# UnaryPlus/raytrace

Measured on AMD Instinct MI355X. Metric: Msamples/s (pixels×spp/s) + achieved HBM GB/s, Cornell-box 600×600, higher is better.
Workload: dtype f64; 1 GPU; cornell 600x600 200spp depth 50; width=600, height=600, spp=200, max_depth=50, parallelism=rows interleaved over 1 GPU(s), row_block 1

## Files before the change

### raytrace_amd/csrc/rt_trace.h

```cpp
#ifndef RT_TRACE_COMMON_H
#define RT_TRACE_COMMON_H
#include <stdint.h>

#include "../../include/rt.h"
#include "rt_internal.h"
#include "rt_sincos_table.h"

#ifdef RT_HOST_EMU
#include <cmath>
#include <cstring>
#define RT_FN static inline
#define RT_FN_SPEC inline
namespace rt_emu {
inline int f2i(float f) {
  int i;
  std::memcpy(&i, &f, 4);
  return i;
}
extern thread_local long long counters[4];
}
#define RT_F2I(f) rt_emu::f2i(f)
#define RT_COUNT(i) (++rt_emu::counters[i])
#define RT_ANY(x) (x)
#define RT_BALLOT_COUNT(x) ((x) ? 1 : 0)
#define RT_CAS
#else
#define RT_FN __device__ __forceinline__
#define RT_FN_SPEC __device__ __forceinline__
#define RT_F2I(f) __float_as_int(f)
#define RT_COUNT(i) ((void)0)
#define RT_ANY(x) __any(x)
#define RT_BALLOT_COUNT(x) ((int)__popcll(__ballot(x)))
#define RT_CAS __attribute__((address_space(4)))
#endif

#ifndef RT_HOOK_SEGMENT
#define RT_HOOK_SEGMENT(pix, sample, seg, R, tbest, best, hit_medium, L, T)
#endif
#ifndef RT_HOOK_SAMPLE
#define RT_HOOK_SAMPLE(pix, sample, L)
#endif
#endif

#ifndef RT_F64
#define RT_F64 0
#endif
#undef RT_NS
#undef RL
#undef RMIN
#undef RMAX
#undef RABS
#undef RFLOOR
#undef RCOPYSIGN
#undef RATAN2
#undef RACOS
#undef RSIN
#undef RFMA
#undef RT_NAN
#undef RT_HUGE
#undef RT_R2I
#undef RT_SINCOS_TURNS
#undef RT_SINCOS_TURNS_S
#undef RT_LOG
#undef RT_RSQRT
#undef RT_RCP
#undef RT_RCP_NZ
#undef RT_SQRT
#undef RT_NODE_F32
#if RT_F64
#define RT_NS rtk64
#define RL(x) x
#define RMIN fmin
#define RMAX fmax
#define RABS fabs
#define RFLOOR floor
#define RCOPYSIGN copysign
#define RATAN2 atan2
#define RACOS acos
#define RSIN sin
#define RFMA fma
#define RT_NAN __builtin_nan("")
#define RT_HUGE __builtin_huge_val()
#define RT_R2I(x) ((int)(uint32_t)__builtin_bit_cast(unsigned long long, (double)(x)))
#define RT_LOG(x) log(x)
#if defined(RT_HOST_EMU) || defined(RT_MATH64_IEEE)
#define RT_SINCOS_TURNS(x, s, c) (*(s) = sin(6.283185307179586 * (x)), *(c) = cos(6.283185307179586 * (x)))
#define RT_RSQRT(x) (1.0 / sqrt(x))
#define RT_RCP(x) (1.0 / (x))
#define RT_RCP_NZ(x) (1.0 / (x))
#define RT_SQRT(x) sqrt(x)
#else
#define RT_SINCOS_TURNS(x, s, c) rt_math64::sincos_turns(x, s, c)
#define RT_SINCOS_TURNS_S(x, s, c) rt_math64::sincos_turns<true>(x, s, c)
#define RT_RSQRT(x) rt_math64::rsqrt(x)
#define RT_RCP(x) rt_math64::rcp(x)
#define RT_RCP_NZ(x) rt_math64::rcp_nz(x)
#define RT_SQRT(x) rt_math64::sqrt_nonneg(x)
#ifndef RT_MATH64_DEFINED
#define RT_MATH64_DEFINED
namespace rt_math64 {
__device__ __forceinline__ double rcp(double x) {
  const double r0 = __builtin_amdgcn_rcp(x);
  const double e = __builtin_fma(-x, r0, 1.0);
  const double r = __builtin_fma(r0, __builtin_fma(e, e, e), r0);
  return r == r ? r : r0;
}
__device__ __forceinline__ double rcp_nz(double x) {
  const double r0 = __builtin_amdgcn_rcp(x);
  const double e = __builtin_fma(-x, r0, 1.0);
  return __builtin_fma(r0, __builtin_fma(e, e, e), r0);
}
__device__ __forceinline__ double rsqrt(double x) {
  const double y = __builtin_amdgcn_rsq(x);
  const double e = __builtin_fma(-x * y, y, 1.0);
  return __builtin_fma(y, __builtin_fma(e, 0.375, 0.5) * e, y);
}
__device__ __forceinline__ double sqrt_nonneg(double x) {
  const double y = __builtin_amdgcn_rsq(x);
  double s = x * y, h = 0.5 * y;
  const double r = __builtin_fma(-s, h, 0.5);
  s = __builtin_fma(s, r, s);
  h = __builtin_fma(h, r, h);
  const double d = __builtin_fma(-s, s, x);
  s = __builtin_fma(d, h, s);
  return x == 0.0 || x == __builtin_huge_val() ? x : s;
}
}
#endif
#endif
#ifndef RT_MATH64_SINCOS_DEFINED
#define RT_MATH64_SINCOS_DEFINED
#ifdef RT_HOST_EMU
#define RT_MATH64_FN static inline
#define RT_MATH64_TAB static
#else
#define RT_MATH64_FN __device__ __forceinline__
#define RT_MATH64_TAB __device__
#endif
namespace rt_math64 {
RT_MATH64_TAB const double rt_sincos_tab[2 * RT_SINCOS_TABLE_N] = RT_SINCOS_TABLE_INIT;
template <bool kCoefScalar = false>
RT_MATH64_FN void sincos_turns(double u, double* sn, double* cs) {
  const double kq = __builtin_rint(u * (double)RT_SINCOS_TABLE_N);
  const double b = __builtin_fma(kq, -1.0 / RT_SINCOS_TABLE_N, u);
  const int k = (int)kq & (RT_SINCOS_TABLE_N - 1);
  const double sa = rt_sincos_tab[2 * k], ca = rt_sincos_tab[2 * k + 1];
  const double x = b * 6.283185307179586, x2 = x * x;
  double c120 = 1.0 / 120.0;
#ifndef RT_HOST_EMU
  if constexpr (kCoefScalar) asm volatile("" : "+s"(c120));
#endif
  double ps = __builtin_fma(x2, -1.0 / 5040.0, c120);
  ps = __builtin_fma(x2, ps, -1.0 / 6.0);
  const double sb = __builtin_fma(x2 * x, ps, x);
  double pc = __builtin_fma(x2, -1.0 / 720.0, 1.0 / 24.0);
  pc = __builtin_fma(x2, pc, -0.5);
  const double cb = __builtin_fma(x2, pc, 1.0);
  *sn = __builtin_fma(sa, cb, ca * sb);
  *cs = __builtin_fma(ca, cb, -(sa * sb));
}
}
#endif
#else
#define RT_NS rtk
#define RL(x) x##f
#define RMIN fminf
#define RMAX fmaxf
#define RABS fabsf
#define RFLOOR floorf
#define RCOPYSIGN copysignf
#define RATAN2 atan2f
#define RACOS acosf
#define RSIN sinf
#define RFMA fmaf
#define RT_NAN __builtin_nanf("")
#define RT_HUGE __builtin_huge_valf()
#define RT_R2I(x) RT_F2I(x)
#ifdef RT_HOST_EMU
#define RT_SINCOS_TURNS(x, s, c) (*(s) = sinf(6.283185307179586f * (x)), *(c) = cosf(6.283185307179586f * (x)))
#define RT_LOG(x) logf(x)
#define RT_RSQRT(x) (1.0f / sqrtf(x))
#define RT_RCP(x) (1.0f / (x))
#define RT_RCP_NZ(x) (1.0f / (x))
#define RT_SQRT(x) sqrtf(x)
#else
#define RT_SINCOS_TURNS(x, s, c) (*(s) = __builtin_amdgcn_sinf(x), *(c) = __builtin_amdgcn_cosf(x))
#define RT_LOG(x) __logf(x)
#define RT_RSQRT(x) __frsqrt_rn(x)
#define RT_RCP(x) __builtin_amdgcn_rcpf(x)
#define RT_RCP_NZ(x) __builtin_amdgcn_rcpf(x)
#define RT_SQRT(x) __builtin_amdgcn_sqrtf(x)
#endif
#endif

namespace RT_NS {

#if RT_F64
using real = double;
using ureal = unsigned long long;
#else
using real = float;
using ureal = uint32_t;
#endif
using KernelParams = ::KernelParamsT<real>;
using DevMaterial = ::DevMaterialT<real>;
using DevTexture = ::DevTextureT<real>;
using DevMedium = ::DevMediumT<real>;
using DevBox = ::DevBoxT<real>;
using DevTarget = ::DevTargetT<real>;
using DevCamera = ::DevCameraT<real>;
using DevInstance = ::DevInstanceT<real>;



constexpr real kPi = RL(3.14159265358979323846);
constexpr real kTmin = RL(0.0001);
constexpr real kInf = RT_HUGE;

#ifdef RT_HOST_EMU
struct alignas(16) v4 {
#else
struct alignas(4 * sizeof(real)) v4 {
#endif
  real x, y, z, w;
};
struct alignas(16) v4f {
  float x, y, z, w;
};
struct alignas(16) i4 {
  int x, y, z, w;
};
struct f3 {
  real x, y, z;
};
RT_FN f3 mk3(real x, real y, real z) { return f3{x, y, z}; }
RT_FN f3 ld3(const real* p) { return f3{p[0], p[1], p[2]}; }
RT_FN f3 operator+(f3 a, f3 b) { return f3{a.x + b.x, a.y + b.y, a.z + b.z}; }
RT_FN f3 operator-(f3 a, f3 b) { return f3{a.x - b.x, a.y - b.y, a.z - b.z}; }
RT_FN f3 operator-(f3 a) { return f3{-a.x, -a.y, -a.z}; }
RT_FN f3 operator*(real s, f3 a) { return f3{s * a.x, s * a.y, s * a.z}; }
RT_FN f3 operator*(f3 a, f3 b) { return f3{a.x * b.x, a.y * b.y, a.z * b.z}; }
RT_FN real dot(f3 a, f3 b) { return a.x * b.x + a.y * b.y + a.z * b.z; }
RT_FN f3 normalize(f3 v) {
  real l = dot(v, v);
#if RT_F64
  if (RABS(l) <= RL(1e-12) || RABS(RL(1.0) - l) <= RL(1e-12)) return v;
#else
  if (l <= RL(1e-12)) return v;
#endif
  return RT_RSQRT(l) * v;
}
RT_FN f3 unit(f3 v) { return RT_RSQRT(dot(v, v)) * v; }
RT_FN f3 reflect(f3 n, f3 v) { return v - (RL(2.0) * dot(n, v)) * n; }
RT_FN f3 xyz(v4 v) { return f3{v.x, v.y, v.z}; }
RT_FN v4 ld4(const real* p) { return *reinterpret_cast<const v4*>(p); }
typedef const RT_CAS real* cfp;
RT_FN cfp cf(const real* p) { return (cfp)p; }
RT_FN f3 ldc3(cfp p) { return f3{p[0], p[1], p[2]}; }
RT_FN v4 ldc4(cfp p) {
  const RT_CAS v4* q = (const RT_CAS v4*)p;
  return v4{q->x, q->y, q->z, q->w};
}
RT_FN int ldci(const int* p, int i) { return ((const RT_CAS int*)p)[i]; }
typedef const RT_CAS float* cfpf;
RT_FN v4f ldc4f(cfpf p) {
  const RT_CAS v4f* q = (const RT_CAS v4f*)p;
  return v4f{q->x, q->y, q->z, q->w};
}

struct u4 {
  uint32_t x, y, z, w;
};
#ifdef RT_HOST_EMU
#define RT_XOR3(a, b, c) ((a) ^ (b) ^ (c))
#else
#define RT_XOR3(a, b, c) __builtin_amdgcn_bitop3_b32((a), (b), (c), 0x96)
#endif
RT_FN u4 philox(uint32_t c0, uint32_t c1, uint32_t c2, uint32_t c3, uint32_t k0, uint32_t k1) {
#ifndef RT_PHILOX_ROUNDS
#define RT_PHILOX_ROUNDS 10
#endif
#ifndef RT_HOST_EMU
  asm volatile("" : "+s"(k0), "+s"(k1));
#endif
#pragma unroll
  for (int r = 0; r < RT_PHILOX_ROUNDS; ++r) {
    if (r) {
      k0 += 0x9E3779B9u;
      k1 += 0xBB67AE85u;
    }
    const uint64_t p0 = (uint64_t)0xD2511F53u * c0, p1 = (uint64_t)0xCD9E8D57u * c2;
    const uint32_t hi0 = (uint32_t)(p0 >> 32), lo0 = (uint32_t)p0;
    const uint32_t hi1 = (uint32_t)(p1 >> 32), lo1 = (uint32_t)p1;
    uint32_t n0 = RT_XOR3(hi1, c1, k0), n2 = RT_XOR3(hi0, c3, k1);
    c0 = n0;
    c1 = lo1;
    c2 = n2;
    c3 = lo0;
  }
  return u4{c0, c1, c2, c3};
}
RT_FN real u01(uint32_t w) { return (real)(w >> 8) * (RL(1.0) / RL(16777216.0)); }

#ifndef RT_SINCOS_TURNS_S
#define RT_SINCOS_TURNS_S RT_SINCOS_TURNS
#endif
template <bool kFlatLoop = false>
RT_FN f3 unit_vector(uint32_t a, uint32_t b) {
  real z = RL(1.0) - RL(2.0) * u01(a);
  real r = RT_SQRT(RMAX(RL(0.0), RL(1.0) - z * z));
  real s, c;
  if constexpr (kFlatLoop)
    RT_SINCOS_TURNS_S(u01(b), &s, &c);
  else
    RT_SINCOS_TURNS(u01(b), &s, &c);
  return mk3(r * c, r * s, z);
}

#if RT_F64 && !defined(RT_NODE_F64)
#define RT_NODE_F32 1
struct f3n {
  float x, y, z;
};
#else
#define RT_NODE_F32 0
#endif
struct RayCtx {
  f3 o, d;
#if RT_NODE_F32
  f3n idir, off0, off1;
#else
  f3 idir, oidir;
#endif
  uint32_t time_w;
  int self_gid;
  int self_inst;
};
template <bool kInst>
RT_FN bool is_self(const RayCtx& R, int gid, int cur_inst) {
  if constexpr (kInst) return gid == R.self_gid && cur_inst == R.self_inst;
  return gid == R.self_gid;
}

RT_FN real u01(uint32_t w);
RT_FN f3 motion_shift(const KernelParams& P, int m, uint32_t time_w) {
  const real time = u01(time_w);
  f3 v0 = ldc3(cf(P.motions) + 8 * m), v1 = ldc3(cf(P.motions) + 8 * m + 4);
  return (RL(1.0) - time) * v0 + time * v1;
}

RT_FN real safe_rcp(real d) { return RT_RCP(RABS(d) > RL(1e-20) ? d : RCOPYSIGN(RL(1e-20), d)); }

#if RT_NODE_F32
#ifndef RT_RCPF
#ifdef RT_HOST_EMU
#define RT_RCPF(x) (1.0f / (x))
#else
#define RT_RCPF(x) __builtin_amdgcn_rcpf(x)
#endif
#endif
RT_FN void prep_axis(real o, real d, float& fi, float& f0, float& f1) {
#ifndef RT_NODE_RCP64
  const float i = RT_RCPF((float)(RABS(d) > RL(1e-20) ? d : RCOPYSIGN(RL(1e-20), d)));
  const float oi = (float)(o * (real)i);
#else
  const real i = safe_rcp(d);
  const float oi = (float)(o * i);
#endif
  const float pad = 3.0e-7f * fabsf(oi);
  const float sp = i >= 0 ? pad : -pad;
  fi = (float)i;
  f0 = oi + sp;
  f1 = oi - sp;
}
RT_FN void prep_ray(RayCtx& R) {
  prep_axis(R.o.x, R.d.x, R.idir.x, R.off0.x, R.off1.x);
  prep_axis(R.o.y, R.d.y, R.idir.y, R.off0.y, R.off1.y);
  prep_axis(R.o.z, R.d.z, R.idir.z, R.off0.z, R.off1.z);
}
RT_FN void node_slabs_f32(const RayCtx& R, const v4f& n0, const v4f& n1, const v4f& n2, float tminf, float ctf,
                          float& lnear, float& lfar, float& rnear, float& rfar) {
  const float lx0 = fmaf(n0.x, R.idir.x, -R.off0.x), lx1 = fmaf(n0.y, R.idir.x, -R.off1.x);
  const float ly0 = fmaf(n0.z, R.idir.y, -R.off0.y), ly1 = fmaf(n0.w, R.idir.y, -R.off1.y);
  const float lz0 = fmaf(n2.x, R.idir.z, -R.off0.z), lz1 = fmaf(n2.y, R.idir.z, -R.off1.z);
  const float rx0 = fmaf(n1.x, R.idir.x, -R.off0.x), rx1 = fmaf(n1.y, R.idir.x, -R.off1.x);
  const float ry0 = fmaf(n1.z, R.idir.y, -R.off0.y), ry1 = fmaf(n1.w, R.idir.y, -R.off1.y);
  const float rz0 = fmaf(n2.z, R.idir.z, -R.off0.z), rz1 = fmaf(n2.w, R.idir.z, -R.off1.z);
  lnear = fmaxf(fmaxf(fminf(lx0, lx1), fminf(ly0, ly1)), fmaxf(fminf(lz0, lz1), tminf));
  lfar = fminf(fminf(fmaxf(lx0, lx1), fmaxf(ly0, ly1)), fminf(fmaxf(lz0, lz1), ctf)) * 1.00000095f;
  rnear = fmaxf(fmaxf(fminf(rx0, rx1), fminf(ry0, ry1)), fmaxf(fminf(rz0, rz1), tminf));
  rfar = fminf(fminf(fmaxf(rx0, rx1), fmaxf(ry0, ry1)), fminf(fmaxf(rz0, rz1), ctf)) * 1.00000095f;
}
#else
RT_FN void prep_ray(RayCtx& R) {
  R.idir = mk3(safe_rcp(R.d.x), safe_rcp(R.d.y), safe_rcp(R.d.z));
  R.oidir = R.o * R.idir;
}
#endif

RT_FN const RT_CAS DevInstance* inst_rec(const KernelParams& P, int k) { return (const RT_CAS DevInstance*)P.instances + k; }
RT_FN f3 inst_to_object(const RT_CAS DevInstance* I, f3 v, bool point) {
  if (point) v = v - mk3(I->m[3], I->m[7], I->m[11]);
  return mk3(I->m[0] * v.x + I->m[4] * v.y + I->m[8] * v.z, I->m[1] * v.x + I->m[5] * v.y + I->m[9] * v.z,
             I->m[2] * v.x + I->m[6] * v.y + I->m[10] * v.z);
}
RT_FN f3 inst_rotate(const RT_CAS DevInstance* I, f3 v) {
  return mk3(I->m[0] * v.x + I->m[1] * v.y + I->m[2] * v.z, I->m[4] * v.x + I->m[5] * v.y + I->m[6] * v.z,
             I->m[8] * v.x + I->m[9] * v.y + I->m[10] * v.z);
}

#if RT_F64
struct Closest {
  real t;
  int ord;
  int prim;
  int inst;
};
#else
struct Closest {
  real t;
  unsigned long long key;
  int prim;
  int inst;
};
#endif
struct Trav {
  int* stack;
  int stride;
  const v4f* lds_nodes;
};
#if RT_F64
RT_FN Closest no_hit() { return Closest{kInf, 0, -1, -1}; }
#else
RT_FN Closest no_hit() { return Closest{kInf, 0x7f80000000000000ull, -1, -1}; }
RT_FN unsigned long long hit_key(real t, int ord) {
  return ((unsigned long long)(unsigned)RT_F2I(t) << 32) | (unsigned)ord;
}
#endif

struct PrimRec {
  v4 a, b, c, e;
};
RT_FN PrimRec ld_rec(cfp pr) { return PrimRec{ldc4(pr), ldc4(pr + 4), ldc4(pr + 8), ldc4(pr + 12)}; }
#ifdef RT_HOST_EMU
#define RT_REC_ALIGN 16
#else
#define RT_REC_ALIGN (16 * sizeof(real))
#endif
struct alignas(RT_REC_ALIGN) PrimRec64 {
  real f[16];
};
RT_FN PrimRec ld_rec64(const RT_CAS PrimRec64* p) {
  const RT_CAS real* r = p->f;
  return PrimRec{v4{r[0], r[1], r[2], r[3]}, v4{r[4], r[5], r[6], r[7]}, v4{r[8], r[9], r[10], r[11]},
                 v4{r[12], r[13], r[14], r[15]}};
}

#if RT_F64
RT_FN real float_up(real x) { return __builtin_bit_cast(real, __builtin_bit_cast(long long, x) + 1); }
#else
RT_FN real float_up(real x) { return __builtin_bit_cast(real, RT_F2I(x) + 1); }
#endif
RT_FN void isect_sphere(const PrimRec& r, f3 o, const RayCtx& R, real tmin, real tmin_up, bool self, real& t,
                        real& q) {
  f3 oc = xyz(r.a) - o;
// ... 609 lines not shown
template <bool kInst, class RC>
RT_FN void test_leaf_generic(const KernelParams& P, RC& R, TravState& S) {
  while (S.leaf < 0) {
    const int enc = ~S.leaf;
    const int first = enc >> RT_LEAF_SHIFT, count = (enc & ((1 << RT_LEAF_SHIFT) - 1)) + 1;
    for (int k = 0; k < count; ++k)
      test_rec<false, kInst>(P, ld_rec(cf(P.prims) + 16 * (size_t)(first + k)), first + k, R, S.tmin, S.tmin_up, S.C,
                             S.inst, S.ord_base);
    S.leaf = 0;
  }
}

template <bool kDefer>
RT_FN void closest_flat(const KernelParams& P, int set, const RayCtx& R, real tmin, Closest& C, real* apdf = nullptr) {
  {
    const DevFlatSet& S = P.flat_sets[set];
    const real tmin_up = float_up(tmin);
    for (int b = S.box_first; b < S.box_end; ++b) test_box<true>((const RT_CAS DevBox*)P.boxes + b, R, tmin_up, C);
    int k = S.first;
    const RT_CAS PrimRec64* rp = (const RT_CAS PrimRec64*)P.flat_recs + k;
    for (; k < S.end_quad; ++k, ++rp) {
      if constexpr (kDefer) {
        if (k == P.target_rec) {
          real term;
          test_static<RT_PRIM_CLASS_QUAD>(ld_rec64(rp), R, tmin, tmin_up, C, 0, &term);
          *apdf = RFMA(P.targets[0].prob_icr, term, *apdf);
          continue;
        }
      }
      test_static<RT_PRIM_CLASS_QUAD>(ld_rec64(rp), R, tmin, tmin_up, C);
    }
    for (; k < S.end_tri; ++k, ++rp) test_static<RT_PRIM_CLASS_TRI>(ld_rec64(rp), R, tmin, tmin_up, C);
    for (; k < S.end_sphere; ++k, ++rp) test_static<RT_PRIM_CLASS_SPHERE>(ld_rec64(rp), R, tmin, tmin_up, C);
    for (; k < S.end; ++k, ++rp) test_rec<true>(P, ld_rec64(rp), k, R, tmin, tmin_up, C);
#if RT_F64
    if (C.t < kInf) C.prim = C.ord;
#else
    const uint32_t hi = (uint32_t)(C.key >> 32);
    if (hi < 0x7f800000u) {
      C.t = __builtin_bit_cast(real, hi);
      C.prim = (int)(uint32_t)C.key;
    }
#endif
  }
}
template <>
RT_FN_SPEC void closest<true>(const KernelParams& P, cfp prims, int root, int set, const RayCtx& R, real tmin, Closest& C,
                         const Trav& W, int* overflow) {
  (void)prims;
  (void)root;
  (void)W;
  (void)overflow;
  closest_flat<false>(P, set, R, tmin, C);
}

template <>
RT_FN_SPEC void closest<false>(const KernelParams& P, cfp prims, int root, int set, const RayCtx& R, real tmin,
                          Closest& C, const Trav& W, int* overflow) {
  TravState S;
  trav_begin(S, root, tmin);
  if (set == 0) prefix_hits(P, prims, R, tmin, S.C);
  while (!trav_done(S)) trav_round(P, R, S, W, *overflow RT_PROF_NULLARG);
  C = S.C;
}

#ifndef RT_KARGS_OPAQUE
#define RT_KARGS_OPAQUE 1
#endif
#if defined(RT_HOST_EMU) || !RT_KARGS_OPAQUE
#define RT_KARGS(P0) (P0)
#else
RT_FN const KernelParams& rt_kargs() {
  const RT_CAS KernelParams* pp = (const RT_CAS KernelParams*)__builtin_amdgcn_kernarg_segment_ptr();
  asm volatile("" : "+s"(pp));
  return *(const KernelParams*)pp;
}
#define RT_KARGS(P0) rt_kargs()
#endif
#ifndef RT_KARGS_TRAV
#define RT_KARGS_TRAV RT_F64
#endif
#define RT_KARGS_IF(on, P0) ((on) ? RT_KARGS(P0) : (P0))

RT_FN uint32_t fast_div(uint32_t n, const FastDiv& f) {
  if (f.d == 1u) return n;
  const uint32_t t = (uint32_t)(((uint64_t)n * f.m) >> 32);
  return (t + ((n - t) >> 1)) >> f.s;
}
RT_FN void camera_ray(const KernelParams& P, uint32_t pix, int sample, uint32_t pxgy, RayCtx& R) {
  int gy, px;
  if (pxgy == ~0u) {
    gy = (int)fast_div(pix, P.div_width);
    px = (int)pix - gy * P.cam.width;
  } else {
    gy = (int)(pxgy >> 16);
    px = (int)(pxgy & 0xffffu);
  }
  u4 w0 = philox(pix, (uint32_t)sample, 0u, RT_EV_CAMERA0, P.key0, P.key1);
  R.time_w = w0.z;
  f3 origin = ld3(P.cam.center);
  if (P.cam.disk_u[0] != RL(0.0) || P.cam.disk_u[1] != RL(0.0) || P.cam.disk_u[2] != RL(0.0) || P.cam.disk_v[0] != RL(0.0) ||
      P.cam.disk_v[1] != RL(0.0) || P.cam.disk_v[2] != RL(0.0)) {
    u4 w1 = philox(pix, (uint32_t)sample, 0u, RT_EV_CAMERA1, P.key0, P.key1);
    real rad = RT_SQRT(u01(w0.w)), s, c;
    RT_SINCOS_TURNS(u01(w1.x), &s, &c);
    origin = origin + (rad * c) * ld3(P.cam.disk_u) + (rad * s) * ld3(P.cam.disk_v);
  }
  f3 target = ld3(P.cam.top_left) + ((real)px + u01(w0.x)) * ld3(P.cam.pixel_u) +
              ((real)gy + u01(w0.y)) * ld3(P.cam.pixel_v);
  R.o = origin;
  R.d = normalize(target - origin);
  R.self_gid = -1;
  R.self_inst = -1;
}

RT_FN void medium_draw(const KernelParams& P, int m, u4 wm, real lo, real hi, real& tbest, int& hit_medium) {
#ifndef RT_HOST_EMU
#pragma clang fp contract(off)
#endif
  uint32_t wsel = (m & 3) == 0 ? wm.x : (m & 3) == 1 ? wm.y : (m & 3) == 2 ? wm.z : wm.w;
  real rnd = RL(1.0) - u01(wsel);
  real hit_dist = P.media[m].neg_inv_density * RT_LOG(rnd);
  if (hit_dist < hi - lo) {
    real t = lo + hit_dist;
    if (t < tbest) {
      tbest = t;
      hit_medium = m;
    }
  }
}
RT_FN u4 medium_block(const KernelParams& P, int m, uint32_t pix, int sample, int seg) {
  return philox(pix, (uint32_t)sample, (uint32_t)seg, RT_EV_MEDIA + (uint32_t)(m >> 2), P.key0, P.key1);
}
RT_FN void medium_event(const KernelParams& P, int m, uint32_t pix, int sample, int seg, real lo, real hi,
                        real& tbest, int& hit_medium) {
  medium_draw(P, m, medium_block(P, m, pix, sample, seg), lo, hi, tbest, hit_medium);
}

template <bool kMats, bool kEarly, class... Defer>
RT_FN bool mixture_scatter(const KernelParams& P, const HitInfo& h, const RayCtx& R, const u4& w, const DevMaterial& Mt,
                           bool hemi, f3 tex, f3& newdir, f3& Tf, Defer... apdf) {
  constexpr bool kDefer = sizeof...(Defer) == 1;
  real cr = u01(w.x);
  int choice = -1;
  for (int k = 0; k < P.n_targets; ++k) {
    if (cr < P.targets[k].thresh) {
      choice = k;
      break;
    }
  }
  f3 dir;
  if constexpr (kDefer) {
    if (choice < 0) {
      dir = h.n + unit_vector<true>(w.y, w.z);
    } else {
      const DevTarget& Tg = P.targets[choice];
      f3 lp = ld3(Tg.q) + u01(w.y) * ld3(Tg.u) + u01(w.z) * ld3(Tg.v);
      dir = lp - h.p;
    }
    dir = normalize(dir);
  } else if (choice < 0) {
    f3 uu = unit_vector(w.y, w.z);
    dir = hemi ? normalize(h.n + uu) : uu;
  } else {
    const DevTarget& Tg = P.targets[choice];
    f3 lp = ld3(Tg.q) + u01(w.y) * ld3(Tg.u) + u01(w.z) * ld3(Tg.v);
    dir = normalize(lp - h.p);
  }
  real pdf1 = hemi ? dot(dir, h.n) * (RL(1.0) / kPi) : RL(0.25) / kPi;
  if constexpr (kEarly)
    if (hemi && pdf1 <= RL(0.0)) return false;
  if constexpr (kDefer && !kMats && !kEarly) {
    if (P.target_defer) {
      *(apdf, ...) = P.rem_prob * pdf1;
      Tf = pdf1 * tex;
      newdir = dir;
      return !(hemi && pdf1 <= RL(0.0));
    }
  }
  real mix = RL(0.0);
  for (int k = 0; k < P.n_targets; ++k) {
    real tt, rinv;
    if (target_hit(P.targets[k], h.p, dir, tt, rinv)) mix += P.targets[k].prob_icr * (tt * tt * RABS(rinv));
  }
  real pdf = P.rem_prob * pdf1 + mix;
  f3 f = tex;
  if constexpr (kMats) {
    if (Mt.kind == 3) {
      real mu0 = -dot(R.d, h.n), mu1 = dot(dir, h.n);
      f = (RL(0.25) * RT_RCP(mu0 + mu1)) * f;
    } else if (Mt.kind == 9) {
      real g = Mt.param, mu = dot(R.d, dir);
      real base = RL(1.0) + g * g - RL(2.0) * g * mu;
      f = ((RL(1.0) - g * g) * RT_RCP(base * RT_SQRT(base))) * f;
    }
  }
  Tf = (pdf1 * RT_RCP(pdf)) * f;
  newdir = dir;
  return !(hemi && pdf1 <= RL(0.0));
}

template <int kTex, bool kMats, bool kInst, class... Defer>
RT_FN bool shade_event(const KernelParams& P, cfp prims, uint32_t pix, int sample, int seg, real tbest, int best,
                       int hit_medium, const RayCtx& R, f3& L, const f3& T, int best_inst, f3& np, f3& nd, f3& Tf,
                       int& ngid, Defer... apdf) {
  RT_HOOK_SEGMENT(pix, sample, seg, R, tbest, best, hit_medium, L, T);
  if (hit_medium < 0 && best < 0) {
    f3 bg = ld3(P.cam.bg0);
    if (P.cam.bg_kind == 1) {
      real a = RL(0.5) * (R.d.y + RL(1.0));
      bg = (RL(1.0) - a) * bg + a * ld3(P.cam.bg1);
    }
    L = L + T * bg;
#ifndef RT_HOST_EMU
    Tf = bg;
#endif
    return true;
  }
  bool terminate = false;
  const RT_CAS DevMaterial* Mp = hit_medium >= 0
                                     ? (const RT_CAS DevMaterial*)P.mats + P.media[hit_medium].material
                                     : (const RT_CAS DevMaterial*)P.prim_shade + best;
  if constexpr (kInst) {
    if (hit_medium < 0 && best_inst >= 0) {
      const int im = inst_rec(P, best_inst)->material;
      if (im >= 0) Mp = (const RT_CAS DevMaterial*)P.mats + im;
    }
  }
  const DevMaterial Mt = DevMaterial{Mp->kind, Mp->tex, Mp->param, Mp->tex_const, {RL(0.), RL(0.), RL(0.)}, RL(0.)};
  const bool need_tex = kTex > 0 && !Mt.tex_const && Mt.kind != RT_MAT_PITCH_BLACK && Mt.kind != RT_MAT_DIELECTRIC;
  HitInfo h;
  if (hit_medium >= 0) {
    h.p = R.o + tbest * R.d;
    h.n = -R.d;
    h.front = true;
    h.u = RL(0.);
    h.v = RL(0.);
    h.gid = -1;
  } else {
    if constexpr (kInst) {
      if (best_inst >= 0) {
        const RT_CAS DevInstance* I = inst_rec(P, best_inst);
        RayCtx Ro = R;
        Ro.o = inst_to_object(I, R.o, true);
        Ro.d = inst_to_object(I, R.d, false);
        h = surface_info(P, prims, best, Ro, tbest, need_tex);
        h.p = R.o + tbest * R.d;
        h.n = inst_rotate(I, h.n);
      } else {
        h = surface_info(P, prims, best, R, tbest, need_tex);
      }
    } else {
      h = surface_info(P, prims, best, R, tbest, need_tex);
    }
  }
  f3 tex = f3{Mp->c0[0], Mp->c0[1], Mp->c0[2]};
  if (need_tex) tex = eval_texture<kTex == 2>(P, Mt.tex, h.u, h.v, h.p);
  u4 w = philox(pix, (uint32_t)sample, (uint32_t)seg, RT_EV_SCATTER, P.key0, P.key1);
#ifdef RT_HOST_EMU
  f3 newdir = mk3(RT_NAN, RT_NAN, RT_NAN);
#elif defined(RT_SHADE_UNDEF)
  f3 newdir;
#else
  f3 newdir = R.d;
  Tf = tex;
#endif
  if constexpr (!kMats) {
    if (Mt.kind == 0) L = L + T * tex;
    terminate = !mixture_scatter<false, false>(P, h, R, w, Mt, true, tex, newdir, Tf, apdf...) || Mt.kind < 2;
  } else {
    switch (Mt.kind) {
      case 0:
        L = L + T * tex;
        terminate = true;
        break;
      case 1:
        terminate = true;
        break;
      case 4:
        Tf = tex;
        newdir = unit(reflect(h.n, R.d));
        break;
      case 5: {
        f3 d2 = reflect(h.n, R.d) + Mt.param * unit_vector(w.y, w.z);
        if (dot(d2, h.n) > RL(0.0)) {
          Tf = tex;
          newdir = normalize(d2);
        } else {
          terminate = true;
        }
        break;
      }
      case 6: {
        Tf = mk3(RL(1.), RL(1.), RL(1.));
        real ior = Mt.param;
        real ratio = h.front ? RT_RCP(ior) : ior;
        real cos_t = RMIN(RL(1.0), -dot(h.n, R.d));
        real sin_t = RT_SQRT(RMAX(RL(0.0), RL(1.0) - cos_t * cos_t));
        real r0 = (RL(1.0) - ratio) * RT_RCP(RL(1.0) + ratio);
        r0 = r0 * r0;
        real x1 = RL(1.0) - cos_t, x2 = x1 * x1;
        real reflectance = r0 + (RL(1.0) - r0) * (x2 * x2 * x1);
        if (ratio * sin_t > RL(1.0) || u01(w.x) < reflectance) {
          newdir = unit(reflect(h.n, R.d));
        } else {
          f3 perp = ratio * (R.d + cos_t * h.n);
          newdir = unit(perp - RT_SQRT(RABS(RL(1.0) - dot(perp, perp))) * h.n);
        }
        break;
      }
      case 7:
        Tf = tex;
        newdir = R.d;
        break;
      default:
        terminate = !mixture_scatter<true, true>(P, h, R, w, Mt, Mt.kind == 2 || Mt.kind == 3, tex, newdir, Tf);
        break;
    }
  }
  np = h.p;
  nd = newdir;
  ngid = h.gid;
  return terminate;
}
template <int kTex, bool kMats, bool kInst = false, class... Defer>
RT_FN bool shade(const KernelParams& P, cfp prims, uint32_t pix, int sample, int& seg, real tbest, int best,
                 int hit_medium, RayCtx& R, f3& L, f3& T, int best_inst = -1, Defer... apdf) {
#ifdef RT_HOST_EMU
  const real nan = RT_NAN;
  f3 np = mk3(nan, nan, nan), nd = np, Tf = np;
  int ngid = RT_EMPTY_ROOT;
#elif defined(RT_SHADE_UNDEF)
  f3 np, nd, Tf;
  int ngid;
#else
  f3 np = R.o, nd = R.d, Tf = mk3(RL(1.), RL(1.), RL(1.));
  int ngid = R.self_gid;
#endif
  const bool term =
      shade_event<kTex, kMats, kInst>(P, prims, pix, sample, seg, tbest, best, hit_medium, R, L, T, best_inst, np, nd, Tf,
                                      ngid, apdf...);
  R.o = np;
  R.d = nd;
  T = T * Tf;
  R.self_gid = ngid;
  if constexpr (kInst) R.self_inst = hit_medium >= 0 ? -1 : best_inst;
  const bool cont = !term && seg + 1 < P.cam.max_depth;
  ++seg;
  return !cont;
}

struct ItemCtx {
  int tp;
  int sample, s_end;
  uint32_t pix;
  uint32_t pxgy;
};
template <bool kTwoSizes>
RT_FN bool open_item(const KernelParams& P, int item, ItemCtx& I) {
  const int W = P.cam.width;
  const bool big = kTwoSizes && item < P.big_items;
  const int id = kTwoSizes && !big ? item - P.big_items : item;
  const int n = big ? P.n_big_chunks : P.n_chunks;
  I.tp = (int)fast_div((uint32_t)id, big ? P.div_big : P.div_small);
  const int k = id - I.tp * n;
  const int tr = (int)fast_div((uint32_t)I.tp, P.div_width);
  const int px = I.tp - tr * W;
  const int tb = (int)fast_div((uint32_t)tr, P.div_block);
  const int gy = (tb * P.n_shards + P.shard) * P.row_block + (tr - tb * P.row_block);
  I.pix = (uint32_t)(gy * W + px);
  I.pxgy = (uint32_t)gy << 16 | (uint32_t)px;
  const int chunk = big ? P.big_chunk : P.chunk;
  I.sample = P.sample0 + (big || !kTwoSizes ? 0 : P.small_start) + k * chunk;
  const int last = P.sample0 + P.cam.spp;
  I.s_end = I.sample + chunk < last ? I.sample + chunk : last;
  if (gy >= P.cam.height || P.cam.max_depth <= 0) I.s_end = I.sample;
  return I.sample < I.s_end;
}

#ifndef RT_TAIL_STEAL
#define RT_TAIL_STEAL 1
#endif
#ifndef RT_TAIL_STEAL_BVH
#define RT_TAIL_STEAL_BVH 1
#endif
#if (RT_TAIL_STEAL || RT_TAIL_STEAL_BVH) && !defined(RT_HOST_EMU)
RT_FN bool steal_sample(bool thief, ItemCtx& I, int tp_plain) {
  unsigned long long tm = __ballot(thief);
  unsigned long long vm = __ballot(!thief && I.tp != -1 && I.s_end - I.sample >= 2);
  const int lane = (int)__lane_id();
  bool got = false;
  while (tm != 0ull && vm != 0ull) {
    const int t = __ffsll(tm) - 1, v = __ffsll(vm) - 1;
    tm &= tm - 1ull;
    vm &= vm - 1ull;
    const int s_end = __builtin_amdgcn_readlane(I.s_end, v);
    const int tp = __builtin_amdgcn_readlane(tp_plain, v);
    const uint32_t pix = (uint32_t)__builtin_amdgcn_readlane((int)I.pix, v);
    const uint32_t pxgy = (uint32_t)__builtin_amdgcn_readlane((int)I.pxgy, v);
    if (lane == t) {
      I.tp = tp;
      I.sample = s_end - 1;
      I.s_end = s_end;
      I.pix = pix;
      I.pxgy = pxgy;
      got = true;
    }
    if (lane == v) I.s_end = s_end - 1;
  }
  return got;
}
#endif

RT_FN void camera_ray_flat(const KernelParams& P, uint32_t pix, int sample, uint32_t pxgy, RayCtx& R) {
  const int gy = (int)(pxgy >> 16), px = (int)(pxgy & 0xffffu);
  u4 w0 = philox(pix, (uint32_t)sample, 0u, RT_EV_CAMERA0, P.key0, P.key1);
  R.time_w = w0.z;
  f3 origin = ld3(P.cam.center);
  if (P.cam_defocus) {
    u4 w1 = philox(pix, (uint32_t)sample, 0u, RT_EV_CAMERA1, P.key0, P.key1);
    real rad = RT_SQRT(u01(w0.w)), s, c;
    RT_SINCOS_TURNS_S(u01(w1.x), &s, &c);
    origin = origin + (rad * c) * ld3(P.cam.disk_u) + (rad * s) * ld3(P.cam.disk_v);
  }
  f3 target = ld3(P.cam.top_left) + ((real)px + u01(w0.x)) * ld3(P.cam.pixel_u) +
              ((real)gy + u01(w0.y)) * ld3(P.cam.pixel_v);
  R.o = origin;
  R.d = normalize(target - origin);
  R.self_gid = -1;
  R.self_inst = -1;
}

template <bool kFlat, int kTex, bool kMedia, bool kMats, class Work, class AccT>
RT_FN int lane_loop_lockstep(const KernelParams& P0_, Work& work, const Trav& TW, const real* prims_, AccT& acc) {
#ifdef RT_HOST_EMU
  KernelParams Pm = P0_;
  if constexpr (kFlat && !kMedia && !kMats) rt_host_match_records(Pm);
  const KernelParams& P0 = Pm;
#else
  const KernelParams& P0 = P0_;
#endif
  (void)P0;
  const cfp prims = cf(prims_);
  int overflow = 0;
  ItemCtx I{-1, 0, 0, 0u, 0u};
  int seg = 0;
  acc_clear(acc);
  bool bad = false;
  bool alive = false;
  f3 T = mk3(RL(1.), RL(1.), RL(1.));
  constexpr bool kDefer = kFlat && !kMedia && !kMats;
  real apdf = RL(1.);
  RayCtx R;
  R.o = R.d = mk3(RL(0.), RL(0.), RL(0.));
#if RT_NODE_F32
  R.idir = R.off0 = R.off1 = f3n{0.f, 0.f, 0.f};
#else
  R.idir = R.oidir = R.o;
#endif
  R.time_w = 0u;
  R.self_gid = -1;
  R.self_inst = -1;
  RT_PROF_DECL
  for (;;) {
    const KernelParams& P = RT_KARGS(P0);
    const bool need = !alive && I.sample >= I.s_end;
    RT_PROF_ADD(PF_ITERS, 1);
    RT_PROF_ADD(PF_FRONT_LANES, RT_BALLOT_COUNT(need));
    work.commit(need && I.tp != -1, I.tp, acc, bad);
    int aslot;
    const int got = work.grab(need, aslot);
#if RT_TAIL_STEAL && !defined(RT_HOST_EMU)
    bool stolen = false;
    if constexpr (kFlat) {
      const bool thief = need && got >= P.n_items;
      if (RT_ANY(thief)) stolen = steal_sample(thief, I, work.untag(I.tp));
    }
#else
    const bool stolen = false;
#endif
    if (need) {
      if (got >= P.n_items && !stolen) break;
      acc_clear(acc);
      bad = false;
      if (!stolen) {
        const bool ok = open_item<kFlat>(P, got, I);
        I.tp = work.tag(I.tp, aslot);
        if (!ok) continue;
      }
    }
    RT_PROF_MARK(PF_FRONT);
    RT_PROF_ADD(PF_CAM_LANES, RT_BALLOT_COUNT(!alive));
    if (!alive) {
      if constexpr (kFlat)
        camera_ray_flat(P, I.pix, I.sample, I.pxgy, R);
      else
        camera_ray(P, I.pix, I.sample, I.pxgy, R);
      T = mk3(RL(1.), RL(1.), RL(1.));
      seg = 0;
      alive = true;
    }
    RT_PROF_MARK(PF_CAM);
    RT_COUNT(2);
    if constexpr (!kFlat) prep_ray(R);
    Closest C = no_hit();
    if constexpr (kDefer) {
      closest_flat<true>(P, 0, R, kTmin, C, &apdf);
      if (P.target_defer) T = (seg == 0 ? RL(1.) : RT_RCP(apdf)) * T;
    } else {
      closest<kFlat>(P, prims, P.surface_root, 0, R, kTmin, C, TW, &overflow);
    }
    real tbest = C.t;
    const int best = C.prim;
    int hit_medium = -1;
    const int n_media = kMedia ? P.n_media : 0;
    for (int m = 0; m < n_media; ++m) {
      const DevMedium& M = P.media[m];
      Closest C1 = no_hit();
      if (M.alias_surface) {
        C1.t = C.t;
        C1.prim = C.prim;
      } else {
        closest<kFlat>(P, prims, M.root, m + 1, R, kTmin, C1, TW, &overflow);
      }
      if (C1.prim < 0) continue;
      const real t1 = C1.t;
      real lo, hi;
      if (prim_front(P, prims, C1.prim, R, t1)) {
        if (!(t1 < tbest)) continue;
        Closest C2 = no_hit();
        closest<kFlat>(P, prims, M.root, m + 1, R, t1, C2, TW, &overflow);
        if (C2.prim < 0) continue;
        lo = t1;
        hi = C2.t;
      } else {
        lo = kTmin;
        hi = t1;
      }
      medium_event(P, m, I.pix, I.sample, seg, lo, hi, tbest, hit_medium);
    }
    RT_PROF_MARK(PF_TRAV);
    f3 L = mk3(RL(0.), RL(0.), RL(0.));
    bool ended;
    if constexpr (kDefer)
      ended = shade<kTex, kMats, false>(P, prims, I.pix, I.sample, seg, tbest, best, hit_medium, R, L, T, -1, &apdf);
    else
      ended = shade<kTex, kMats>(P, prims, I.pix, I.sample, seg, tbest, best, hit_medium, R, L, T);
    if (ended) {
#ifdef RT_HOST_EMU
      apdf = RT_NAN;
#endif
      RT_HOOK_SAMPLE(I.pix, I.sample, L);
      acc_sample(acc, L, bad);
      alive = false;
      ++I.sample;
    }
    RT_PROF_MARK(PF_SHADE);
  }
  RT_PROF_FLUSH
  return overflow;
}

template <bool kInst>
RT_FN void media_events_late(const KernelParams& P, cfp prims, const RayCtx& R, uint32_t pix, int sample, int seg, int best,
                             real t_surf, real& tbest, int& hit_medium) {
  for (int m = 0; m < P.n_media; ++m) {
    const DevMedium& M = P.media[m];
    bool ev = false;
    real lo = kTmin, hi = t_surf;
    if (M.alias_surface) {
      ev = best >= 0 && !prim_front(P, prims, best, R, t_surf);
    } else {
      const int enc = ~M.root;
      const int first = enc >> RT_LEAF_SHIFT, end = first + (enc & ((1 << RT_LEAF_SHIFT) - 1)) + 1;
      Closest C1 = no_hit();
      for (int k = first; k < end; ++k)
        test_rec<false, kInst>(P, ld_rec64((const RT_CAS PrimRec64*)prims + k), k, R, kTmin, float_up(kTmin), C1);
      if (C1.prim >= 0) {
        const real t1 = C1.t;
        if (prim_front(P, prims, C1.prim, R, t1)) {
          if (t1 < tbest) {
            Closest C2 = no_hit();
            for (int k = first; k < end; ++k)
              test_rec<false, kInst>(P, ld_rec64((const RT_CAS PrimRec64*)prims + k), k, R, t1, float_up(t1), C2);
            ev = C2.prim >= 0;
            lo = t1;
            hi = C2.t;
// ... 178 lines not shown
```

Baseline: 16590 Msamples/s.

## Add restart-at-generate lane loop merging camera and scatter ray generation

Adds a specialized lane loop for flat, untextured, media-free, material-free scenes. A terminated path restarts at the ray-generation step in the same iteration, so camera rays and scatter rays share a single philox call, a single normalize and a single traversal step, which should reduce divergence between lanes on different path stages. It also adds a sincos variant that pins three polynomial coefficients in scalar registers. The restructuring changes control flow and adds code-path complexity, and the scalar-register pinning may shift register allocation.

```diff
diff --git a/raytrace_amd/csrc/rt_trace.h b/raytrace_amd/csrc/rt_trace.h
--- a/raytrace_amd/csrc/rt_trace.h
+++ b/raytrace_amd/csrc/rt_trace.h
@@ -61,6 +61,7 @@
 #undef RT_R2I
 #undef RT_SINCOS_TURNS
 #undef RT_SINCOS_TURNS_S
+#undef RT_SINCOS_TURNS_S2
 #undef RT_LOG
 #undef RT_RSQRT
 #undef RT_RCP
@@ -91,7 +92,8 @@
 #define RT_SQRT(x) sqrt(x)
 #else
 #define RT_SINCOS_TURNS(x, s, c) rt_math64::sincos_turns(x, s, c)
-#define RT_SINCOS_TURNS_S(x, s, c) rt_math64::sincos_turns<true>(x, s, c)
+#define RT_SINCOS_TURNS_S(x, s, c) rt_math64::sincos_turns<1>(x, s, c)
+#define RT_SINCOS_TURNS_S2(x, s, c) rt_math64::sincos_turns<2>(x, s, c)
 #define RT_RSQRT(x) rt_math64::rsqrt(x)
 #define RT_RCP(x) rt_math64::rcp(x)
 #define RT_RCP_NZ(x) rt_math64::rcp_nz(x)
@@ -139,21 +141,22 @@
 #endif
 namespace rt_math64 {
 RT_MATH64_TAB const double rt_sincos_tab[2 * RT_SINCOS_TABLE_N] = RT_SINCOS_TABLE_INIT;
-template <bool kCoefScalar = false>
+template <int kCoefScalar = 0>
 RT_MATH64_FN void sincos_turns(double u, double* sn, double* cs) {
   const double kq = __builtin_rint(u * (double)RT_SINCOS_TABLE_N);
   const double b = __builtin_fma(kq, -1.0 / RT_SINCOS_TABLE_N, u);
   const int k = (int)kq & (RT_SINCOS_TABLE_N - 1);
   const double sa = rt_sincos_tab[2 * k], ca = rt_sincos_tab[2 * k + 1];
   const double x = b * 6.283185307179586, x2 = x * x;
-  double c120 = 1.0 / 120.0;
+  double c120 = 1.0 / 120.0, c6 = -1.0 / 6.0, c24 = 1.0 / 24.0;
 #ifndef RT_HOST_EMU
-  if constexpr (kCoefScalar) asm volatile("" : "+s"(c120));
+  if constexpr (kCoefScalar == 1) asm volatile("" : "+s"(c120));
+  if constexpr (kCoefScalar == 2) asm volatile("" : "+s"(c120), "+s"(c6), "+s"(c24));
 #endif
   double ps = __builtin_fma(x2, -1.0 / 5040.0, c120);
-  ps = __builtin_fma(x2, ps, -1.0 / 6.0);
+  ps = __builtin_fma(x2, ps, c6);
   const double sb = __builtin_fma(x2 * x, ps, x);
-  double pc = __builtin_fma(x2, -1.0 / 720.0, 1.0 / 24.0);
+  double pc = __builtin_fma(x2, -1.0 / 720.0, c24);
   pc = __builtin_fma(x2, pc, -0.5);
   const double cb = __builtin_fma(x2, pc, 1.0);
   *sn = __builtin_fma(sa, cb, ca * sb);
@@ -305,12 +308,17 @@
 #ifndef RT_SINCOS_TURNS_S
 #define RT_SINCOS_TURNS_S RT_SINCOS_TURNS
 #endif
-template <bool kFlatLoop = false>
+#ifndef RT_SINCOS_TURNS_S2
+#define RT_SINCOS_TURNS_S2 RT_SINCOS_TURNS
+#endif
+template <int kFlatLoop = 0>
 RT_FN f3 unit_vector(uint32_t a, uint32_t b) {
   real z = RL(1.0) - RL(2.0) * u01(a);
   real r = RT_SQRT(RMAX(RL(0.0), RL(1.0) - z * z));
   real s, c;
-  if constexpr (kFlatLoop)
+  if constexpr (kFlatLoop == 2)
+    RT_SINCOS_TURNS_S2(u01(b), &s, &c);
+  else if constexpr (kFlatLoop == 1)
     RT_SINCOS_TURNS_S(u01(b), &s, &c);
   else
     RT_SINCOS_TURNS(u01(b), &s, &c);
@@ -1226,7 +1234,7 @@
   f3 dir;
   if constexpr (kDefer) {
     if (choice < 0) {
-      dir = h.n + unit_vector<true>(w.y, w.z);
+      dir = h.n + unit_vector<1>(w.y, w.z);
     } else {
       const DevTarget& Tg = P.targets[choice];
       f3 lp = ld3(Tg.q) + u01(w.y) * ld3(Tg.u) + u01(w.z) * ld3(Tg.v);
@@ -1505,8 +1513,195 @@
   R.self_inst = -1;
 }
 
+#ifndef RT_RESTART_AT_GENERATE
+#define RT_RESTART_AT_GENERATE 1
+#endif
+template <class Work, class AccT>
+RT_FN int lane_loop_restart(const KernelParams& P0_, Work& work, const real* prims_, AccT& acc) {
+#ifdef RT_HOST_EMU
+  KernelParams Pm = P0_;
+  rt_host_match_records(Pm);
+  const KernelParams& P0 = Pm;
+#else
+  const KernelParams& P0 = P0_;
+#endif
+  (void)P0;
+  const cfp prims = cf(prims_);
+  ItemCtx I{-1, 0, 0, 0u, 0u};
+  int seg = 0;
+  acc_clear(acc);
+  bool bad = false;
+  bool alive = false;
+  f3 T = mk3(RL(1.), RL(1.), RL(1.));
+  real apdf = RL(1.);
+  RayCtx R;
+  R.o = R.d = mk3(RL(0.), RL(0.), RL(0.));
+#if RT_NODE_F32
+  R.idir = R.off0 = R.off1 = f3n{0.f, 0.f, 0.f};
+#else
+  R.idir = R.oidir = R.o;
+#endif
+  R.time_w = 0u;
+  R.self_gid = -1;
+  R.self_inst = -1;
+  RT_PROF_DECL
+  for (;;) {
+    const KernelParams& P = RT_KARGS(P0);
+    RT_PROF_ADD(PF_ITERS, 1);
+    bool restart = true;
+#ifdef RT_HOST_EMU
+    f3 hp = mk3(RT_NAN, RT_NAN, RT_NAN), hn = hp, tex = hp;
+#else
+    f3 hp = R.o, hn = R.d, tex = T;
+#endif
+    if (alive) {
+      RT_COUNT(2);
+      Closest C = no_hit();
+      closest_flat<true>(P, 0, R, kTmin, C, &apdf);
+      if (P.target_defer) T = (seg == 0 ? RL(1.) : RT_RCP(apdf)) * T;
+      const real tbest = C.t;
+      const int best = C.prim;
+      RT_PROF_MARK(PF_TRAV);
+      f3 L = mk3(RL(0.), RL(0.), RL(0.));
+      RT_HOOK_SEGMENT(I.pix, I.sample, seg, R, tbest, best, -1, L, T);
+      if (best < 0) {
+        f3 bg = ld3(P.cam.bg0);
+        if (P.cam.bg_kind == 1) {
+          real a = RL(0.5) * (R.d.y + RL(1.0));
+          bg = (RL(1.0) - a) * bg + a * ld3(P.cam.bg1);
+        }
+        L = L + T * bg;
+      } else {
+        const RT_CAS DevMaterial* Mp = (const RT_CAS DevMaterial*)P.prim_shade + best;
+        const int kind = Mp->kind;
+        const HitInfo h = surface_info(P, prims, best, R, tbest, false);
+        tex = f3{Mp->c0[0], Mp->c0[1], Mp->c0[2]};
+        if (kind == 0) L = L + T * tex;
+        hp = h.p;
+        hn = h.n;
+        R.self_gid = h.gid;
+        restart = kind < 2 || seg + 1 >= P.cam.max_depth;
+      }
+      if (restart) {
+        RT_HOOK_SAMPLE(I.pix, I.sample, L);
+        acc_sample(acc, L, bad);
+        ++I.sample;
+        alive = false;
+#ifdef RT_HOST_EMU
+        R.o = R.d = T = mk3(RT_NAN, RT_NAN, RT_NAN);
+        apdf = RT_NAN;
+        R.self_gid = R.self_inst = RT_EMPTY_ROOT;
+#endif
+      }
+      RT_PROF_MARK(PF_SHADE);
+    }
+    const bool need = restart && I.sample >= I.s_end;
+    RT_PROF_ADD(PF_FRONT_LANES, RT_BALLOT_COUNT(need));
+    work.commit(need && I.tp != -1, I.tp, acc, bad);
+    int aslot;
+    const int got = work.grab(need, aslot);
+#if RT_TAIL_STEAL && !defined(RT_HOST_EMU)
+    bool stolen = false;
+    const bool thief = need && got >= P.n_items;
+    if (RT_ANY(thief)) stolen = steal_sample(thief, I, work.untag(I.tp));
+#else
+    const bool stolen = false;
+#endif
+    if (need) {
+      if (got >= P.n_items && !stolen) break;
+      acc_clear(acc);
+      bad = false;
+      if (!stolen) {
+        const bool ok = open_item<true>(P, got, I);
+        I.tp = work.tag(I.tp, aslot);
+        if (!ok) continue;
+      }
+    }
+    RT_PROF_MARK(PF_FRONT);
+    RT_PROF_ADD(PF_CAM_LANES, RT_BALLOT_COUNT(restart));
+    const u4 w = philox(I.pix, (uint32_t)I.sample, restart ? 0u : (uint32_t)seg,
+                        restart ? (uint32_t)RT_EV_CAMERA0 : (uint32_t)RT_EV_SCATTER, P.key0, P.key1);
+    f3 org, dir;
+    if (restart) {
+      const int gy = (int)(I.pxgy >> 16), px = (int)(I.pxgy & 0xffffu);
+      R.time_w = w.z;
+      org = ld3(P.cam.center);
+      if (P.cam_defocus) {
+        u4 w1 = philox(I.pix, (uint32_t)I.sample, 0u, RT_EV_CAMERA1, P.key0, P.key1);
+        real rad = RT_SQRT(u01(w.w)), s, c;
+        RT_SINCOS_TURNS_S2(u01(w1.x), &s, &c);
+        org = org + (rad * c) * ld3(P.cam.disk_u) + (rad * s) * ld3(P.cam.disk_v);
+      }
+      f3 target = ld3(P.cam.top_left) + ((real)px + u01(w.x)) * ld3(P.cam.pixel_u) +
+                  ((real)gy + u01(w.y)) * ld3(P.cam.pixel_v);
+      dir = target - org;
+    } else {
+      real cr = u01(w.x);
+      int choice = -1;
+      for (int k = 0; k < P.n_targets; ++k) {
+        if (cr < P.targets[k].thresh) {
+          choice = k;
+          break;
+        }
+      }
+      if (choice < 0) {
+        dir = hn + unit_vector<2>(w.y, w.z);
+      } else {
+        const DevTarget& Tg = P.targets[choice];
+        f3 lp = ld3(Tg.q) + u01(w.y) * ld3(Tg.u) + u01(w.z) * ld3(Tg.v);
+        dir = lp - hp;
+      }
+      org = hp;
+    }
+    dir = normalize(dir);
+    R.o = org;
+    R.d = dir;
+    if (restart) {
+      R.self_gid = -1;
+      R.self_inst = -1;
+      T = mk3(RL(1.), RL(1.), RL(1.));
+      seg = 0;
+      alive = true;
+    } else {
+      const real pdf1 = dot(dir, hn) * (RL(1.0) / kPi);
+      f3 Tf;
+      if (P.target_defer) {
+        apdf = P.rem_prob * pdf1;
+        Tf = pdf1 * tex;
+      } else {
+        real mix = RL(0.0);
+        for (int k = 0; k < P.n_targets; ++k) {
+          real tt, rinv;
+          if (target_hit(P.targets[k], hp, dir, tt, rinv)) mix += P.targets[k].prob_icr * (tt * tt * RABS(rinv));
+        }
+        real pdf = P.rem_prob * pdf1 + mix;
+        Tf = (pdf1 * RT_RCP(pdf)) * tex;
+      }
+      T = T * Tf;
+      ++seg;
+      if (pdf1 <= RL(0.0)) {
+        const f3 zero = mk3(RL(0.), RL(0.), RL(0.));
+        RT_HOOK_SAMPLE(I.pix, I.sample, zero);
+        acc_sample(acc, zero, bad);
+        ++I.sample;
+        alive = false;
+#ifdef RT_HOST_EMU
+        R.o = R.d = T = mk3(RT_NAN, RT_NAN, RT_NAN);
+        apdf = RT_NAN;
+        R.self_gid = R.self_inst = RT_EMPTY_ROOT;
+#endif
+      }
+    }
+    RT_PROF_MARK(PF_CAM);
+  }
+  RT_PROF_FLUSH
+  return 0;
+}
+
 template <bool kFlat, int kTex, bool kMedia, bool kMats, class Work, class AccT>
 RT_FN int lane_loop_lockstep(const KernelParams& P0_, Work& work, const Trav& TW, const real* prims_, AccT& acc) {
+  if constexpr (RT_RESTART_AT_GENERATE && kFlat && kTex == 0 && !kMedia && !kMats)
+    return lane_loop_restart(P0_, work, prims_, acc);
 #ifdef RT_HOST_EMU
   KernelParams Pm = P0_;
   if constexpr (kFlat && !kMedia && !kMats) rt_host_match_records(Pm);
```

Result: no change. 16710 Msamples/s (median of 6 runs) (+0.7%).
